# supranational/sppark

Hardware: NVIDIA H100
Metric: BLS12-381 G1 MSM/s @2^26 points (higher is better)
Workload: dtype u32x12 (384-bit Montgomery integers)

## Files before the change

### sppark_b200/csrc/msm/msm.cuh

```cuda
#pragma once
#include "../util/gpu.cuh"
#include "msm_core.cuh"
#include "msm_pair.cuh"
#include "msm_table.cuh"

namespace msm {

#ifndef SPPARK_B200_ACC_THREADS
# define SPPARK_B200_ACC_THREADS 128
#endif
#ifndef SPPARK_B200_ACC_MIN_BLOCKS
# define SPPARK_B200_ACC_MIN_BLOCKS 3
#endif
constexpr uint32_t ACC_THREADS = SPPARK_B200_ACC_THREADS;
constexpr uint32_t HEAVY_THREADS = 128;

constexpr uint32_t HIST_THREADS = 1024;
constexpr uint32_t HIST_SMEM_WORDS = 56 * 1024;
constexpr uint32_t SORT_THREADS = 512;
constexpr uint32_t SORT_CAP = 24576;

template<class Load, class Visit>
__device__ uint32_t block_exclusive_scan(uint32_t len, Load load, Visit visit)
{
    __shared__ uint32_t warp_tot[32];
    const uint32_t lane = threadIdx.x & 31, wid = threadIdx.x >> 5, nw = blockDim.x >> 5;
    uint32_t carry = 0;
    for (uint32_t t0 = 0; t0 < len; t0 += 4 * blockDim.x) {
        const uint32_t b = t0 + 4 * threadIdx.x;
        uint32_t c[4];
#pragma unroll
        for (uint32_t k = 0; k < 4; k++) c[k] = b + k < len ? load(b + k) : 0;
        const uint32_t s = c[0] + c[1] + c[2] + c[3];
        uint32_t x = s;
#pragma unroll
        for (uint32_t d = 1; d < 32; d <<= 1) {
            const uint32_t y = __shfl_up_sync(0xffffffffu, x, d);
            if (lane >= d) x += y;
        }
        if (lane == 31) warp_tot[wid] = x;
        __syncthreads();
        if (wid == 0) {
            uint32_t t = lane < nw ? warp_tot[lane] : 0;
#pragma unroll
            for (uint32_t d = 1; d < 32; d <<= 1) {
                const uint32_t y = __shfl_up_sync(0xffffffffu, t, d);
                if (lane >= d) t += y;
            }
            warp_tot[lane] = t;
        }
        __syncthreads();
        uint32_t r = carry + (wid ? warp_tot[wid - 1] : 0) + x - s;
        carry += warp_tot[31];
#pragma unroll
        for (uint32_t k = 0; k < 4; k++) {
            if (b + k < len) visit(b + k, c[k], r);
            r += c[k];
        }
        __syncthreads();
    }
    return carry;
}

static __global__ void __launch_bounds__(HIST_THREADS)
bin_hist_kernel(const Config cfg, uint32_t lg_bins, const uint32_t* scalars, uint32_t wpg, uint32_t* bin_count)
{
    extern __shared__ uint32_t hist[];
    const uint32_t w0 = blockIdx.y * wpg, w1 = min(w0 + wpg, cfg.nwins), nctr = (w1 - w0) << lg_bins;
    const uint32_t d_end = cfg.copies > 1 ? digit_count(cfg) : w1;
    const uint32_t lane = threadIdx.x & 31;
    for (uint32_t k = threadIdx.x; k < nctr; k += blockDim.x) hist[k] = 0;
    __syncthreads();
    for (uint32_t i0 = blockIdx.x * blockDim.x + (threadIdx.x & ~31u); i0 < cfg.npoints; i0 += gridDim.x * blockDim.x) {
        const uint32_t i = i0 + lane;
        for_each_digit(cfg, lg_bins, scalars, i, i < cfg.npoints, d_end,
                       [&](uint32_t w, bool nz, uint32_t bin, uint32_t, uint32_t) {
            if (w < w0 || w >= w1) return;
            const uint32_t key = nz ? bin - (w0 << lg_bins) : ~0u;
            const uint32_t peers = __match_any_sync(0xffffffffu, key);
            if (nz && lane == __ffs(peers) - 1) atomicAdd(&hist[key], __popc(peers));
        });
    }
    __syncthreads();
    for (uint32_t k = threadIdx.x; k < nctr; k += blockDim.x)
        if (hist[k]) atomicAdd(&bin_count[((size_t)w0 << lg_bins) + k], hist[k]);
}

static __global__ void __launch_bounds__(1024)
bin_scan_kernel(uint32_t lg_bins, const uint32_t* bin_count, uint32_t* bin_base, uint32_t* bin_cur)
{
    const size_t row = (size_t)blockIdx.x << lg_bins;
    block_exclusive_scan(1u << lg_bins, [&](uint32_t j) { return bin_count[row + j]; },
                         [&](uint32_t j, uint32_t, uint32_t off) { bin_base[row + j] = off; bin_cur[row + j] = off; });
}

static __global__ void __launch_bounds__(256)
partition_kernel(const Config cfg, uint32_t lg_bins, const uint32_t* scalars, uint32_t* bin_cur, uint2* staging)
{
    const uint32_t lane = threadIdx.x & 31;
    for (uint32_t i0 = blockIdx.x * blockDim.x + (threadIdx.x & ~31u); i0 < cfg.npoints; i0 += gridDim.x * blockDim.x) {
        const uint32_t i = i0 + lane;
        for_each_digit(cfg, lg_bins, scalars, i, i < cfg.npoints, digit_count(cfg),
                       [&](uint32_t w, bool nz, uint32_t bin, uint32_t b, uint32_t entry) {
            const uint32_t peers = __match_any_sync(0xffffffffu, nz ? bin : ~0u);
            const uint32_t leader = __ffs(peers) - 1;
            uint32_t pos = 0;
            if (nz && lane == leader) pos = atomicAdd(&bin_cur[bin], __popc(peers));
            pos = __shfl_sync(0xffffffffu, pos, leader) + __popc(peers & ((1u << lane) - 1));
            if (nz) staging[(size_t)w * row_stride(cfg) + pos] = make_uint2(entry, b);
        });
    }
}

static __global__ void __launch_bounds__(SORT_THREADS)
bin_sort_kernel(const Config cfg, uint32_t lg_bins, uint32_t cap, const uint2* staging, const uint32_t* bin_count,
                const uint32_t* bin_base, uint32_t* counts, uint32_t* offsets, uint32_t* sorted, uint32_t* ctrl,
                uint32_t* heavy_list, uint32_t* chunk_map, uint32_t* overflow)
{
    extern __shared__ uint32_t sm[];
    const uint32_t w = blockIdx.x >> lg_bins, bin = blockIdx.x & ((1u << lg_bins) - 1);
    uint32_t b0, nbk;
    if (!bin_buckets(cfg, lg_bins, w, bin, b0, nbk)) return;
    const uint32_t cnt = bin_count[blockIdx.x], base = bin_base[blockIdx.x];
    const size_t t0 = ((size_t)w << cfg.lg_nb) + b0;
    if (last_bin(cfg, lg_bins, w, bin))
        for (uint32_t b = b0 + nbk + threadIdx.x; b < (1u << cfg.lg_nb); b += blockDim.x)
            offsets[((size_t)w << cfg.lg_nb) + b] = base + cnt;
    if (cnt > cap) {
        if (threadIdx.x == 0) overflow[atomicAdd(&ctrl[3], 1)] = blockIdx.x;
        return;
    }
    uint32_t *run = sm, *cur = sm + cap;
    for (uint32_t k = threadIdx.x; k < nbk; k += blockDim.x) cur[k] = 0;
    __syncthreads();
    const uint2* src = staging + (size_t)w * row_stride(cfg) + base;
    for (uint32_t k = threadIdx.x; k < cnt; k += blockDim.x) atomicAdd(&cur[src[k].y - b0], 1);
    __syncthreads();
    block_exclusive_scan(nbk, [&](uint32_t j) { return cur[j]; }, [&](uint32_t j, uint32_t c, uint32_t off) {
        counts[t0 + j] = c;
        offsets[t0 + j] = base + off;
        cur[j] = off;
        register_heavy(cfg, (uint32_t)(t0 + j), c, ctrl, heavy_list, chunk_map);
    });
    for (uint32_t k = threadIdx.x; k < cnt; k += blockDim.x) {
        const uint2 e = src[k];
        run[atomicAdd(&cur[e.y - b0], 1)] = e.x;
    }
    __syncthreads();
    uint32_t* dst = sorted + (size_t)w * row_stride(cfg) + base;
    for (uint32_t k = threadIdx.x; k < cnt; k += blockDim.x) dst[k] = run[k];
}

template<bool PLACE>
__global__ void __launch_bounds__(256)
overflow_kernel(const Config cfg, uint32_t lg_bins, const uint2* staging, const uint32_t* bin_count,
                const uint32_t* bin_base, const uint32_t* ctrl, const uint32_t* overflow, uint32_t* slots,
                uint32_t* sorted)
{
    const uint32_t lane = threadIdx.x & 31, nov = ctrl[3];
    for (uint32_t o = 0; o < nov; o++) {
        const uint32_t g = overflow[o], w = g >> lg_bins, cnt = bin_count[g];
        const uint2* src = staging + (size_t)w * row_stride(cfg) + bin_base[g];
        uint32_t* row = slots + ((size_t)w << cfg.lg_nb);
        for (uint32_t k0 = blockIdx.x * blockDim.x + (threadIdx.x & ~31u); k0 < cnt; k0 += gridDim.x * blockDim.x) {
            const uint32_t k = k0 + lane;
            const uint2 e = k < cnt ? src[k] : make_uint2(0, ~0u);
            const uint32_t peers = __match_any_sync(0xffffffffu, e.y);
            const uint32_t leader = __ffs(peers) - 1;
            uint32_t pos = 0;
            if (k < cnt && lane == leader) pos = atomicAdd(&row[e.y], __popc(peers));
            if (PLACE) {
                pos = __shfl_sync(0xffffffffu, pos, leader) + __popc(peers & ((1u << lane) - 1));
                if (k < cnt) sorted[(size_t)w * row_stride(cfg) + pos] = e.x;
            }
        }
    }
}

static __global__ void __launch_bounds__(1024)
overflow_scan_kernel(const Config cfg, uint32_t lg_bins, const uint32_t* bin_base, const uint32_t* overflow,
                     const uint32_t* counts, uint32_t* offsets, uint32_t* cursor, uint32_t* ctrl,
                     uint32_t* heavy_list, uint32_t* chunk_map)
{
    const uint32_t nov = ctrl[3];
    for (uint32_t o = blockIdx.x; o < nov; o += gridDim.x) {
        const uint32_t g = overflow[o], w = g >> lg_bins, base = bin_base[g];
        uint32_t b0, nbk;
        bin_buckets(cfg, lg_bins, w, g & ((1u << lg_bins) - 1), b0, nbk);
        const size_t t0 = ((size_t)w << cfg.lg_nb) + b0;
        block_exclusive_scan(nbk, [&](uint32_t j) { return counts[t0 + j]; }, [&](uint32_t j, uint32_t c, uint32_t off) {
            offsets[t0 + j] = base + off;
            cursor[t0 + j] = base + off;
            register_heavy(cfg, (uint32_t)(t0 + j), c, ctrl, heavy_list, chunk_map);
        });
    }
}

struct SortBufs {
    uint32_t *counts, *offsets, *cursor, *ctrl, *heavy_list, *chunk_map, *sorted;
    uint32_t *bin_count, *bin_base, *bin_cur, *overflow;
    uint2* staging;
};

inline bool sort_profile() { const char* e = getenv("SPPARK_B200_MSM_SORT_PROFILE"); return e && atoi(e) != 0; }

inline void sort_slice(const Config& cfg, uint32_t cap, const uint32_t* d_scalars, const SortBufs& s, uint32_t sms,
                       cudaStream_t stream)
{
    const uint32_t lg_bins = sort_lg_bins(cfg, row_stride(cfg));
    const size_t nbins = (size_t)cfg.nwins << lg_bins, nslots = (size_t)cfg.nwins << cfg.lg_nb;
    const bool marks = sort_profile();
    CUDA_OK(cudaFuncSetAttribute(bin_hist_kernel, cudaFuncAttributeMaxDynamicSharedMemorySize, HIST_SMEM_WORDS * 4));
    CUDA_OK(cudaFuncSetAttribute(bin_sort_kernel, cudaFuncAttributeMaxDynamicSharedMemorySize,
                                 (SORT_CAP + (1u << SORT_SMAX)) * 4));
    CUDA_OK(cudaMemsetAsync(s.counts, 0, nslots * 4, stream));
    CUDA_OK(cudaMemsetAsync(s.ctrl, 0, 16, stream));
    CUDA_OK(cudaMemsetAsync(s.bin_count, 0, nbins * 4, stream));
    const uint32_t wpg = std::min(cfg.nwins, HIST_SMEM_WORDS >> lg_bins);
    const uint32_t ngroups = (cfg.nwins + wpg - 1) / wpg;
    const uint32_t hist_blk = (uint32_t)std::min<size_t>((cfg.npoints + HIST_THREADS - 1) / HIST_THREADS, sms);
    bin_hist_kernel<<<dim3(hist_blk, ngroups), HIST_THREADS, ((size_t)wpg << lg_bins) * 4, stream>>>(
        cfg, lg_bins, d_scalars, wpg, s.bin_count);
    COUNT_LAUNCH();
    bin_scan_kernel<<<cfg.nwins, 1024, 0, stream>>>(lg_bins, s.bin_count, s.bin_base, s.bin_cur);
    COUNT_LAUNCH();
    if (marks) g_profile.mark("sort_partition", stream);
    const uint32_t part_blk = (uint32_t)std::min<size_t>((cfg.npoints + 255) / 256, (size_t)sms * 8);
    partition_kernel<<<part_blk, 256, 0, stream>>>(cfg, lg_bins, d_scalars, s.bin_cur, s.staging);
    COUNT_LAUNCH();
    if (marks) g_profile.mark("sort_bins", stream);
    bin_sort_kernel<<<(uint32_t)nbins, SORT_THREADS, (cap + (1u << SORT_SMAX)) * 4, stream>>>(
        cfg, lg_bins, cap, s.staging, s.bin_count, s.bin_base, s.counts, s.offsets, s.sorted, s.ctrl,
        s.heavy_list, s.chunk_map, s.overflow);
    COUNT_LAUNCH();
    if (marks) g_profile.mark("sort_overflow", stream);
    overflow_kernel<false><<<sms * 4, 256, 0, stream>>>(cfg, lg_bins, s.staging, s.bin_count, s.bin_base, s.ctrl,
                                                        s.overflow, s.counts, s.sorted);
    overflow_scan_kernel<<<sms, 1024, 0, stream>>>(cfg, lg_bins, s.bin_base, s.overflow, s.counts, s.offsets, s.cursor,
                                                   s.ctrl, s.heavy_list, s.chunk_map);
    overflow_kernel<true><<<sms * 4, 256, 0, stream>>>(cfg, lg_bins, s.staging, s.bin_count, s.bin_base, s.ctrl,
                                                       s.overflow, s.cursor, s.sorted);
    COUNT_LAUNCH(); COUNT_LAUNCH(); COUNT_LAUNCH();
    CUDA_OK(cudaGetLastError());
}

static __global__ void pair_counts_kernel(const Config cfg, const uint32_t* counts, uint32_t* counts1, uint32_t nslots)
{
    for (uint32_t t = blockIdx.x * blockDim.x + threadIdx.x; t < nslots; t += gridDim.x * blockDim.x)
        pair_counts_body(cfg, counts, counts1, t);
}

static __global__ void __launch_bounds__(1024)
pair_scan_kernel(const Config cfg, const uint32_t* counts1, uint32_t* off1, uint32_t* wintotal)
{
    __shared__ uint32_t warp_tot[32];
    const uint32_t w = blockIdx.x, nb = 1u << cfg.lg_nb, lane = threadIdx.x & 31, wid = threadIdx.x >> 5;
    const size_t base = (size_t)w << cfg.lg_nb;
    uint32_t carry = 0;
    for (uint32_t t0 = 0; t0 < nb; t0 += 4096) {
        const uint32_t b = t0 + threadIdx.x * 4;
        uint4 c = make_uint4(0, 0, 0, 0);
        if (b < nb) c = *reinterpret_cast<const uint4*>(counts1 + base + b);
        const uint32_t s = c.x + c.y + c.z + c.w;
        uint32_t x = s;
#pragma unroll
        for (uint32_t d = 1; d < 32; d <<= 1) {
            uint32_t y = __shfl_up_sync(0xffffffffu, x, d);
            if (lane >= d) x += y;
        }
        if (lane == 31) warp_tot[wid] = x;
        __syncthreads();
        if (wid == 0) {
            uint32_t t = warp_tot[lane];
#pragma unroll
            for (uint32_t d = 1; d < 32; d <<= 1) {
                uint32_t y = __shfl_up_sync(0xffffffffu, t, d);
                if (lane >= d) t += y;
            }
            warp_tot[lane] = t;
        }
        __syncthreads();
        uint4 r;
        r.x = carry + (wid ? warp_tot[wid - 1] : 0) + x - s;
        r.y = r.x + c.x;
        r.z = r.y + c.y;
        r.w = r.z + c.z;
        carry += warp_tot[31];
        if (b < nb) *reinterpret_cast<uint4*>(off1 + base + b) = r;
        __syncthreads();
    }
    if (threadIdx.x == 0) wintotal[w] = carry;
}

static __global__ void pair_winbase_kernel(const Config cfg, const uint32_t* wintotal, uint32_t* winbase)
{
    if (blockIdx.x || threadIdx.x) return;
    uint32_t run = 0;
    for (uint32_t w = 0; w < cfg.nwins; w++) { winbase[w] = run; run += wintotal[w]; }
    winbase[cfg.nwins] = run;
}

template<class F>
__global__ void __launch_bounds__(128)
pair_forward_kernel(const Config cfg, const uint32_t* points, const uint32_t* sorted, const uint32_t* offsets,
                    const uint32_t* counts, const uint32_t* counts1, const uint32_t* off1, const uint32_t* winbase,
                    uint32_t o0, uint32_t nthreads, uint32_t* pre, uint32_t* totals)
{
    const uint32_t tid = blockIdx.x * blockDim.x + threadIdx.x;
    if (tid < nthreads)
        pair_forward_body<F>(cfg, points, sorted, offsets, counts, counts1, off1, winbase, o0, nthreads, pre, totals, tid);
}

// ... 249 lines not shown
finish_par_kernel(const Config cfg, const uint32_t* winR, uint32_t* out_jacobian)
{
    __shared__ F slots[Par4<F>::NS];
    if (threadIdx.x >= 4) return;
    Par4<F> p(slots, slots + 4, threadIdx.x);
    {
        const ec::xyzz_t<F> top = load_bucket<F>(winR, cfg.nwins - 1);
        if (p.lane == 0) { slots[Par4<F>::sX] = top.X; slots[Par4<F>::sY] = top.Y; slots[Par4<F>::sZZZ] = top.ZZZ; slots[Par4<F>::sZZ] = top.ZZ; }
        p.sync();
    }
    for (uint32_t w = cfg.nwins - 1; w-- > 0;) {
        for (uint32_t d = 0; d < cfg.wbits; d++) p.dbl();
        p.add(load_bucket<F>(winR, w));
    }
    const bool inf = p.is_inf();
    const F ZZ = slots[Par4<F>::sZZ];
    const F Yf = slots[Par4<F>::sY], ZZZf = slots[Par4<F>::sZZZ];
    const F r = F::mul_shared(p.pick(slots[Par4<F>::sX], Yf, Yf, Yf), p.pick(ZZ, ZZZf, ZZZf, ZZZf));
    if (p.lane < 2)
        for (int k = 0; k < F::N; k++) out_jacobian[p.lane * F::N + k] = inf ? 0 : r.l[k];
    if (p.lane == 2)
        for (int k = 0; k < F::N; k++) out_jacobian[2 * F::N + k] = inf ? 0 : ZZ.l[k];
}

static __global__ void pack_points_kernel(const uint8_t* in, size_t stride, uint32_t words, bool has_flag,
                                   uint32_t* out, uint32_t npoints)
{
    for (uint32_t i = blockIdx.x * blockDim.x + threadIdx.x; i < npoints; i += gridDim.x * blockDim.x) {
        const uint32_t* src = reinterpret_cast<const uint32_t*>(in + (size_t)i * stride);
        bool inf = has_flag && (in[(size_t)i * stride + 4 * words] & 1);
        for (uint32_t k = 0; k < words; k++) out[(size_t)i * words + k] = inf ? 0 : src[k];
    }
}

template<class F>
__global__ void __launch_bounds__(128)
table_double_kernel(const uint32_t* packed, size_t first, uint32_t n, uint32_t steps, uint32_t copies,
                    uint32_t* xyzz, uint32_t* zzz)
{
    const uint32_t i = blockIdx.x * blockDim.x + threadIdx.x;
    if (i < n) table_double_body<F>(packed, first, n, steps, copies, xyzz, zzz, i);
}

template<class F>
__global__ void __launch_bounds__(128)
table_normalize_kernel(const uint32_t* xyzz, const uint32_t* zzz_inv, size_t npoints, size_t first, uint32_t n,
                       uint32_t nslots, uint32_t* table)
{
    const uint32_t s = blockIdx.x * blockDim.x + threadIdx.x;
    if (s < nslots) table_normalize_body<F>(xyzz, zzz_inv, npoints, first, n, table, s);
}

template<class F>
void build_table(uint32_t* d_table, size_t npoints, const Config& cfg, const stream_t& stream)
{
    const uint32_t K1 = cfg.copies - 1, steps = cfg.wbits * cfg.nwins;
    if (K1 == 0 || npoints == 0) return;
    const size_t chunk = std::min<size_t>(npoints, ((size_t)1 << 21) / K1);
    dev_ptr_t<uint32_t> xyzz(chunk * K1 * 4 * F::N, stream), zzz(chunk * K1 * F::N, stream);
    for (size_t first = 0; first < npoints; first += chunk) {
        const uint32_t n = (uint32_t)std::min(chunk, npoints - first), ns = n * K1;
        table_double_kernel<F><<<(n + 127) / 128, 128, 0, stream>>>(d_table, first, n, steps, cfg.copies, xyzz, zzz);
        pair_invert_kernel<F><<<((ns + PAIR_M - 1) / PAIR_M + 127) / 128, 128, 0, stream>>>(zzz, ns);
        table_normalize_kernel<F><<<(ns + 127) / 128, 128, 0, stream>>>(xyzz, zzz, npoints, first, n, ns, d_table);
        COUNT_LAUNCH(); COUNT_LAUNCH(); COUNT_LAUNCH();
        CUDA_OK(cudaGetLastError());
    }
}

template<class F>
class msm_t {
    const gpu_t& gpu;
    static constexpr uint32_t PW = 2 * F::N, BW = 4 * F::N, JW = 3 * F::N;

public:
    explicit msm_t(const gpu_t& g) : gpu(g) {}

    struct Job {
        Config cfg;
        size_t nslots, slice_cap;
        uint32_t lg_l, items1;
        uint8_t* blob;
        uint32_t *counts, *offsets, *cursor, *ctrl, *heavy_list, *chunk_map, *partials, *sorted, *buckets;
        uint32_t *bin_count, *bin_base, *bin_cur, *overflow;
        uint2* staging;
        uint32_t *R[2], *S[2];
        uint32_t slices_done;
        bool pair;
        size_t pair_bound;
        uint32_t pair_threads;
        uint32_t *counts1, *off1, *wintotal, *winbase, *sums, *pre, *totals;
        cudaStream_t owner;
        Job() : blob(nullptr), owner(nullptr) {}
        Job(const Job&) = delete;
        Job& operator=(const Job&) = delete;
        Job(Job&& o) noexcept { memcpy((void*)this, (const void*)&o, sizeof(Job)); o.blob = nullptr; }
        ~Job() { if (blob) (void)cudaFreeAsync(blob, owner); }
    };

    Job begin(size_t total_points, size_t slice_cap, cudaStream_t stream)
    {
        if (total_points >= (1ull << 31))
            throw cuda_error(-(int)cudaErrorInvalidValue, "msm: npoints must be < 2^31");
        return begin(make_config(total_points), slice_cap, stream);
    }

    Job begin(const Config& cfg, size_t slice_cap, cudaStream_t stream)
    {
        Job j;
        j.cfg = cfg;
        j.cfg.npoints = (uint32_t)slice_cap;
        j.slice_cap = slice_cap;
        j.nslots = (size_t)j.cfg.nwins << j.cfg.lg_nb;
        j.lg_l = j.cfg.lg_nb > 12 ? j.cfg.lg_nb - 12 : 0;
        j.items1 = j.cfg.nwins << (j.cfg.lg_nb - j.lg_l);
        j.slices_done = 0;
        const size_t entries = (size_t)j.cfg.nwins * row_stride(j.cfg);
        const size_t heavy_cap = entries / (j.cfg.heavy + 1) + 1;
        const size_t chunk_cap = entries / j.cfg.heavy_chunk + heavy_cap;
        size_t off = 0;
        auto take = [&](size_t bytes) { size_t o = off; off += (bytes + 255) & ~(size_t)255; return o; };
        const size_t o_counts = take(j.nslots * 4), o_offsets = take(j.nslots * 4), o_cursor = take(j.nslots * 4);
        const size_t nbins = (size_t)j.cfg.nwins << sort_lg_bins(j.cfg, row_stride(j.cfg));
        const size_t o_bcount = take(nbins * 4), o_bbase = take(nbins * 4), o_bcur = take(nbins * 4), o_over = take(nbins * 4);
        const size_t o_staging = take(entries * 8);
        const size_t o_ctrl = take(16), o_heavy = take(heavy_cap * 12), o_cmap = take(chunk_cap * 4);
        const size_t o_partials = take(chunk_cap * BW * 4);
        const size_t o_sorted = take(entries * 4);
        const size_t o_buckets = take(j.nslots * BW * 4);
        const size_t o_r0 = take((size_t)j.items1 * BW * 4), o_s0 = take((size_t)j.items1 * BW * 4);
        const size_t o_r1 = take((size_t)j.items1 * BW * 4 / 2 + 4096), o_s1 = take((size_t)j.items1 * BW * 4 / 2 + 4096);
        const char* pair_env = getenv("SPPARK_B200_MSM_PAIR");
        j.pair = pair_env && atoi(pair_env) != 0 && entries + j.nslots < (1ull << 31);
        j.pair_bound = (entries + std::min<size_t>(entries, j.nslots) + 1) / 2;
        j.pair_threads = (uint32_t)std::min<size_t>((j.pair_bound + PAIR_K - 1) / PAIR_K, (size_t)1 << 21);
        size_t o_c1 = 0, o_o1 = 0, o_wt = 0, o_wb = 0, o_sums = 0, o_pre = 0, o_tot = 0;
        if (j.pair) {
            o_c1 = take(j.nslots * 4); o_o1 = take(j.nslots * 4);
            o_wt = take((j.cfg.nwins + 1) * 4); o_wb = take((j.cfg.nwins + 1) * 4);
            o_sums = take(j.pair_bound * 2 * F::N * 4);
            o_pre = take((size_t)j.pair_threads * PAIR_K * F::N * 4);
            o_tot = take((size_t)j.pair_threads * F::N * 4);
        }
        CUDA_OK(cudaMallocAsync((void**)&j.blob, off, stream));
        j.owner = stream;
        auto U32 = [&](size_t o) { return reinterpret_cast<uint32_t*>(j.blob + o); };
        j.counts = U32(o_counts); j.offsets = U32(o_offsets); j.cursor = U32(o_cursor);
        j.ctrl = U32(o_ctrl); j.heavy_list = U32(o_heavy); j.chunk_map = U32(o_cmap);
        j.partials = U32(o_partials); j.sorted = U32(o_sorted); j.buckets = U32(o_buckets);
        j.bin_count = U32(o_bcount); j.bin_base = U32(o_bbase); j.bin_cur = U32(o_bcur); j.overflow = U32(o_over);
        j.staging = reinterpret_cast<uint2*>(j.blob + o_staging);
        j.R[0] = U32(o_r0); j.S[0] = U32(o_s0); j.R[1] = U32(o_r1); j.S[1] = U32(o_s1);
        j.counts1 = U32(o_c1); j.off1 = U32(o_o1); j.wintotal = U32(o_wt); j.winbase = U32(o_wb);
        j.sums = U32(o_sums); j.pre = U32(o_pre); j.totals = U32(o_tot);
        g_profile.reset();
        return j;
    }

    void slice(Job& j, const uint32_t* d_points, const uint32_t* d_scalars, size_t n, cudaStream_t stream)
    {
        if (n == 0) return;
        Config cfg = j.cfg;
        cfg.npoints = (uint32_t)n;
        cfg.merge = j.slices_done ? 1 : 0;
        const uint32_t sms = (uint32_t)gpu.sm_count();
        g_profile.mark("sort", stream);
        const SortBufs sb{j.counts, j.offsets, j.cursor, j.ctrl, j.heavy_list, j.chunk_map, j.sorted,
                          j.bin_count, j.bin_base, j.bin_cur, j.overflow, j.staging};
        sort_slice(cfg, SORT_CAP, d_scalars, sb, sms, stream);

        g_profile.mark("accumulate", stream);
        int occ = 1;
        CUDA_OK(cudaOccupancyMaxActiveBlocksPerMultiprocessor(&occ, accumulate_kernel<F>, ACC_THREADS, 0));
        if (occ < 1) occ = 1;
        size_t want = (j.nslots + ACC_THREADS - 1) / ACC_THREADS;
        uint32_t acc_blocks = (uint32_t)std::min<size_t>(want, (size_t)sms * occ);
        if (j.pair) {
            const uint32_t nslots = (uint32_t)j.nslots;
            pair_counts_kernel<<<sms * 8, 256, 0, stream>>>(cfg, j.counts, j.counts1, nslots);
            pair_scan_kernel<<<cfg.nwins, 1024, 0, stream>>>(cfg, j.counts1, j.off1, j.wintotal);
            pair_winbase_kernel<<<1, 32, 0, stream>>>(cfg, j.wintotal, j.winbase);
            const size_t ent = (size_t)cfg.nwins * row_stride(cfg);
            const size_t bound = (ent + std::min<size_t>(ent, j.nslots) + 1) / 2;
            const size_t per_launch = (size_t)j.pair_threads * PAIR_K;
            for (size_t o0 = 0; o0 < bound; o0 += per_launch) {
                const uint32_t nth = (uint32_t)std::min<size_t>(j.pair_threads, (bound - o0 + PAIR_K - 1) / PAIR_K);
                pair_forward_kernel<F><<<(nth + 127) / 128, 128, 0, stream>>>(
                    cfg, d_points, j.sorted, j.offsets, j.counts, j.counts1, j.off1, j.winbase, (uint32_t)o0, nth, j.pre, j.totals);
                pair_invert_kernel<F><<<((nth + PAIR_M - 1) / PAIR_M + 127) / 128, 128, 0, stream>>>(j.totals, nth);
                pair_backward_kernel<F><<<(nth + 127) / 128, 128, 0, stream>>>(
                    cfg, d_points, j.sorted, j.offsets, j.counts, j.counts1, j.off1, j.winbase, (uint32_t)o0, nth, j.pre, j.totals, j.sums);
                COUNT_LAUNCH(); COUNT_LAUNCH(); COUNT_LAUNCH();
            }
            CUDA_OK(cudaGetLastError());
            g_profile.mark("accumulate_sums", stream);
            accumulate_direct_kernel<F><<<acc_blocks, ACC_THREADS, 0, stream>>>(cfg, j.sums, j.offsets, j.counts, j.buckets,
                                                                               j.ctrl, j.counts1, j.off1, j.winbase);
        } else {
            accumulate_kernel<F><<<acc_blocks, ACC_THREADS, 0, stream>>>(cfg, d_points, j.sorted, j.offsets, j.counts,
                                                                        j.buckets, j.ctrl);
        }
        COUNT_LAUNCH();
        g_profile.mark("heavy", stream);
        heavy_chunks_kernel<F><<<sms * 4, HEAVY_THREADS, HEAVY_THREADS * BW * 4, stream>>>(
            cfg, d_points, j.sorted, j.offsets, j.counts, j.ctrl, j.heavy_list, j.chunk_map, j.partials);
        COUNT_LAUNCH();
        heavy_fold_kernel<F><<<sms, HEAVY_THREADS, HEAVY_THREADS * BW * 4, stream>>>(cfg, j.ctrl, j.heavy_list,
                                                                                    j.partials, j.buckets);
        COUNT_LAUNCH();
        CUDA_OK(cudaGetLastError());
        if (getenv("SPPARK_B200_MSM_DEBUG")) {
            uint32_t dbg[3];
            CUDA_OK(cudaMemcpyAsync(dbg, j.ctrl, 12, cudaMemcpyDeviceToHost, stream));
            CUDA_OK(cudaStreamSynchronize(stream));
            fprintf(stderr, "[msm] slice %u n=%u wbits=%u nwins=%u heavy_thr=%u tasks_claimed=%u nheavy=%u nchunks=%u acc_blocks=%u"
                    " digits=%u sets=%u copies=%u\n",
                    j.slices_done, cfg.npoints, cfg.wbits, cfg.nwins, cfg.heavy, dbg[0], dbg[1], dbg[2], acc_blocks,
                    digit_count(cfg), cfg.nwins, cfg.copies);
        }
        j.slices_done++;
    }

    void finish(Job& j, uint32_t* d_out, cudaStream_t stream)
    {
        if (j.slices_done == 0) {
            CUDA_OK(cudaMemsetAsync(d_out, 0, JW * 4, stream));
        } else {
            const Config& cfg = j.cfg;
            g_profile.mark("reduce", stream);
            reduce1_kernel<F><<<(j.items1 + 127) / 128, 128, 0, stream>>>(cfg, j.buckets, j.lg_l, j.items1, j.R[0], j.S[0]);
            COUNT_LAUNCH();
            uint32_t per_win = 1u << (cfg.lg_nb - j.lg_l), lg_span = j.lg_l, cur = 0;
            while (per_win > 1) {
                uint32_t lg_g = 31 - __builtin_clz(per_win);
                if (lg_g > 4) lg_g = 4;
                uint32_t G = 1u << lg_g, nitems = cfg.nwins * (per_win >> lg_g);
                constexpr uint32_t PG = par_groups<F>::value;
                combine_par_kernel<F><<<(nitems + PG - 1) / PG, 4 * PG, 0, stream>>>(j.R[cur], j.S[cur], G, lg_span, nitems,
                                                                                     j.R[cur ^ 1], j.S[cur ^ 1]);
                COUNT_LAUNCH();
                per_win >>= lg_g;
                lg_span += lg_g;
                cur ^= 1;
            }
            g_profile.mark("finish", stream);
            finish_par_kernel<F><<<1, 32, 0, stream>>>(cfg, j.R[cur], d_out);
            COUNT_LAUNCH();
            g_profile.mark("end", stream);
            CUDA_OK(cudaGetLastError());
        }
        CUDA_OK(cudaFreeAsync(j.blob, stream));
// ... 18 lines not shown
```

### sppark_b200/csrc/msm/msm_bls12_381.cu

```cuda
#include "msm_host.cuh"

RustError msm_host_bls12_381(void* out, const void* points, size_t npoints, const void* scalars,
                             size_t stride, bool has_flag, bool mont)
{
    return msm_host<ff::bls12_381_fp_t>(out, points, npoints, scalars, stride, has_flag,
                                        mont ? scalars_from_mont<ff::bls12_381_fr_t> : nullptr);
}
RustError msm_dev_bls12_381(void* out, const void* d_points, size_t npoints, const void* d_scalars, void* stream)
{   return msm_dev<ff::bls12_381_fp_t>(out, d_points, npoints, d_scalars, stream);   }

RustError gen_points_bls12_381(void* d_out, size_t n, void* stream)
{   return gen_points_dev<ff::bls12_381_g1_gen>(d_out, n, stream);   }
RustError combine_bls12_381(void* out, const void* partials, size_t count)
{   return combine_host<ff::bls12_381_fp_t>(out, partials, count);   }

extern "C" RustError mult_pippenger(void* out, const void* points, size_t npoints, const void* scalars)
{   return msm_host_bls12_381(out, points, npoints, scalars, 96, false, false);   }

extern "C" RustError mult_pippenger_inf(void* out, const void* points, size_t npoints,
                                        const void* scalars, size_t ffi_affine_sz)
{   return msm_host_bls12_381(out, points, npoints, scalars, ffi_affine_sz, true, false);   }

template<class F>
__global__ void selftest_kernel(int op, size_t n, uint32_t* r, const uint32_t* a, const uint32_t* b)
{
    size_t i = blockIdx.x * (size_t)blockDim.x + threadIdx.x;
    if (i >= n) return;
    F x, y, z;
    for (int k = 0; k < F::N; k++) { x.l[k] = a[i * F::N + k]; y.l[k] = b[i * F::N + k]; }
    switch (op) {
    case 0: z = x * y; break;
    case 1: z = x + y; break;
    case 2: z = x - y; break;
    case 3: z = x.sqr(); break;
    case 4: z = F::mul_shared(x, y); break;
    case 5: z = F::sqr_shared(x); break;
    default: z = F::msub_shared(x, y, y, x.sqr()); break;
    }
    for (int k = 0; k < F::N; k++) r[i * F::N + k] = z.l[k];
}

template<class F>
static RustError selftest(int op, size_t n, void* r, const void* a, const void* b)
{
    try {
        const gpu_t& gpu = select_gpu(-1);
        const stream_t& s = gpu[0];
        size_t bytes = n * F::N * 4;
        dev_ptr_t<uint32_t> da(n * F::N, s), db(n * F::N, s), dr(n * F::N, s);
        s.HtoD(da, a, bytes);
        s.HtoD(db, b, bytes);
        selftest_kernel<F><<<(unsigned)((n + 127) / 128), 128, 0, s>>>(op, n, dr, da, db);
        COUNT_LAUNCH();
        CUDA_OK(cudaGetLastError());
        s.DtoH(r, dr, bytes);
        s.sync();
    } catch (const cuda_error& e) {
        return rust_err(e.code(), e.what());
    }
    return rust_ok();
}

extern "C" RustError sppark_b200_selftest_field(int field, int op, size_t n, void* r, const void* a, const void* b)
{
    switch (field) {
    case 0: return selftest<ff::bls12_381_fp_t>(op, n, r, a, b);
    case 1: return selftest<ff::bls12_381_fr_t>(op, n, r, a, b);
    case 2: return selftest<ff::pallas_fp_t>(op, n, r, a, b);
    case 3: return selftest<ff::vesta_fp_t>(op, n, r, a, b);
    case 4: return selftest<ff::bn254_fp_t>(op, n, r, a, b);
    case 5: return selftest<ff::bn254_fr_t>(op, n, r, a, b);
    case 6: return selftest<ff::bls12_377_fp_t>(op, n, r, a, b);
    case 7: return selftest<ff::bls12_377_fr_t>(op, n, r, a, b);
    default: return rust_err(-(int)cudaErrorInvalidValue, "selftest: unknown field");
    }
}

RustError msm_preload_bls12_381(const void* points, size_t npoints, size_t stride, bool has_flag, void** d_points,
                                uint32_t* copies, uint32_t* wbits)
{   return msm_preload<ff::bls12_381_fp_t>(points, npoints, stride, has_flag, d_points, copies, wbits);   }
RustError msm_resident_bls12_381(void* out, const void* d_points, size_t npoints, const void* scalars, bool mont,
                                 uint32_t wbits, uint32_t copies, size_t stride)
{
    return msm_resident<ff::bls12_381_fp_t, ff::bls12_381_fr_t>(out, d_points, npoints, scalars, mont, wbits, copies, stride);
}

extern "C" RustError sppark_b200_selftest_msm_sort(size_t n, uint32_t wbits, uint32_t cap, const void* scalars,
                                                   void* counts, void* offsets, void* sorted, void* heavy_slots,
                                                   uint32_t* info)
{
    using namespace msm;
    if (n == 0 || n >= (1ull << 31) || wbits < 3 || wbits > 24 || cap > SORT_CAP)
        return rust_err(-(int)cudaErrorInvalidValue, "selftest_msm_sort: bad arguments");
    try {
        const gpu_t& gpu = select_gpu(-1);
        const stream_t& s = gpu[0];
        Config cfg = make_config(n);
        cfg.wbits = wbits;
        cfg.nwins = (256 + wbits - 1) / wbits;
        cfg.lg_nb = wbits - 1;
        const size_t nslots = (size_t)cfg.nwins << cfg.lg_nb, entries = (size_t)cfg.nwins * n;
        const size_t nbins = (size_t)cfg.nwins << sort_lg_bins(cfg, n);
        const size_t heavy_cap = entries / (cfg.heavy + 1) + 1, chunk_cap = entries / cfg.heavy_chunk + heavy_cap;
        dev_ptr_t<uint32_t> d_sc(8 * n, s), d_counts(nslots, s), d_offsets(nslots, s), d_cursor(nslots, s);
        dev_ptr_t<uint32_t> d_ctrl(4, s), d_heavy(3 * heavy_cap, s), d_cmap(chunk_cap, s), d_sorted(entries, s);
        dev_ptr_t<uint32_t> d_bcount(nbins, s), d_bbase(nbins, s), d_bcur(nbins, s), d_over(nbins, s);
        dev_ptr_t<uint32_t> d_staging(2 * entries, s);
        s.HtoD(d_sc, scalars, 32 * n);
        const SortBufs sb{d_counts, d_offsets, d_cursor, d_ctrl, d_heavy, d_cmap, d_sorted,
                          d_bcount, d_bbase, d_bcur, d_over, reinterpret_cast<uint2*>((uint32_t*)d_staging)};
        sort_slice(cfg, cap ? cap : SORT_CAP, d_sc, sb, (uint32_t)gpu.sm_count(), s);
        uint32_t ctrl[4];
        s.DtoH(ctrl, d_ctrl, 16);
        s.DtoH(counts, d_counts, nslots * 4);
        s.DtoH(offsets, d_offsets, nslots * 4);
        s.DtoH(sorted, d_sorted, entries * 4);
        s.sync();
        std::vector<uint32_t> hl(3 * (size_t)ctrl[1] + 1);
        if (ctrl[1]) s.DtoH(hl.data(), d_heavy, 12 * (size_t)ctrl[1]);
        s.sync();
        for (uint32_t h = 0; h < ctrl[1]; h++) static_cast<uint32_t*>(heavy_slots)[h] = hl[3 * h];
        info[0] = cfg.nwins; info[1] = cfg.heavy; info[2] = ctrl[1]; info[3] = sort_lg_bins(cfg, n); info[4] = ctrl[3];
    } catch (const cuda_error& e) {
        return rust_err(e.code(), e.what());
    }
    return rust_ok();
}
```

### sppark_b200/csrc/msm/msm_core.cuh

```cuda
#pragma once
#include <algorithm>
#include "../ec/xyzz.cuh"

namespace msm {

struct Config {
    uint32_t wbits;
    uint32_t nwins;
    uint32_t lg_nb;
    uint32_t npoints;
    uint32_t heavy;
    uint32_t heavy_chunk;
    uint32_t merge;
    uint32_t copies;
    uint32_t copy_stride;
};

HD uint32_t digit_count(const Config& cfg) { return (256 + cfg.wbits - 1) / cfg.wbits; }
HD size_t row_stride(const Config& cfg) { return cfg.copies * cfg.npoints; }

HD uint32_t digit_slot(const Config& cfg, uint32_t w, uint32_t i, uint32_t neg, uint32_t& entry)
{
    if (cfg.copies == 1) { entry = i | (neg << 31); return w; }
    const uint32_t k = w / cfg.nwins;
// ... 38 lines not shown
            carry = 1;
            raw = (1u << c) - raw;
        } else {
            neg = 0;
            carry = 0;
        }
        bucket = raw - 1;
        return raw != 0;
    }
};

HD void count_body(const Config& cfg, const uint32_t* scalars, uint32_t* counts, uint32_t i)
{
    Digits d(scalars + 8 * (size_t)i);
    const uint32_t nd = digit_count(cfg);
    for (uint32_t w = 0; w < nd; w++) {
        uint32_t b, neg, entry;
        if (d.next(w, cfg.wbits, b, neg))
            atomic_inc(&counts[((size_t)digit_slot(cfg, w, i, neg, entry) << cfg.lg_nb) + b]);
    }
}

HD void scatter_body(const Config& cfg, const uint32_t* scalars, uint32_t* cursor,
                     uint32_t* sorted, uint32_t i, uint32_t w0, uint32_t w1)
{
    Digits d(scalars + 8 * (size_t)i);
    for (uint32_t w = 0; w < w1; w++) {
        uint32_t b, neg, entry;
        if (d.next(w, cfg.wbits, b, neg) && w >= w0) {
            const uint32_t v = digit_slot(cfg, w, i, neg, entry);
            uint32_t pos = atomic_inc(&cursor[((size_t)v << cfg.lg_nb) + b]);
            sorted[(size_t)v * row_stride(cfg) + pos] = entry;
        }
    }
}

constexpr uint32_t SORT_SMAX = 12;
constexpr uint32_t SORT_LG_FILL = 13;

HD uint32_t top_window_bits(const Config& cfg)
{
    const uint32_t e = 255 - (cfg.nwins - 1) * cfg.wbits;
    return e < cfg.lg_nb ? e : cfg.lg_nb;
}
HD uint32_t window_bits(const Config& cfg, uint32_t w)
{   return w + 1 < cfg.nwins || cfg.copies > 1 ? cfg.lg_nb : top_window_bits(cfg);   }
HD uint32_t bin_shift(const Config& cfg, uint32_t lg_bins, uint32_t w)
{
    const uint32_t ub = window_bits(cfg, w);
    return ub > lg_bins ? ub - lg_bins : 0;
}

inline uint32_t sort_lg_bins(const Config& cfg, size_t n)
{
    int lg_n = 0;
    while (((size_t)1 << lg_n) < n) lg_n++;
    int lb = std::max(std::min(lg_n - (int)SORT_LG_FILL, 15), (int)cfg.lg_nb - (int)SORT_SMAX);
    lb = std::min(lb, (int)cfg.lg_nb);
    return (uint32_t)std::max(lb, 2);
}

HD bool bin_buckets(const Config& cfg, uint32_t lg_bins, uint32_t w, uint32_t bin, uint32_t& b0, uint32_t& nbk)
{
    const uint32_t s = bin_shift(cfg, lg_bins, w), ub = window_bits(cfg, w);
    b0 = bin << s;
    nbk = 1u << s;
    return b0 < (1u << ub);
}

HD bool last_bin(const Config& cfg, uint32_t lg_bins, uint32_t w, uint32_t bin)
{   return ((bin + 1) << bin_shift(cfg, lg_bins, w)) == (1u << window_bits(cfg, w));   }

template<class Fn>
HD void for_each_digit(const Config& cfg, uint32_t lg_bins, const uint32_t* scalars, uint32_t i, bool valid,
                       uint32_t w_end, Fn fn)
{
    Digits d(scalars + 8 * (size_t)(valid ? i : 0));
    for (uint32_t w = 0; w < w_end; w++) {
        uint32_t b, neg, entry;
        const bool nz = d.next(w, cfg.wbits, b, neg) && valid;
        const uint32_t v = digit_slot(cfg, w, i, neg, entry);
        fn(v, nz, (v << lg_bins) + (nz ? b >> bin_shift(cfg, lg_bins, v) : 0), b, entry);
    }
}

HD void register_heavy(const Config& cfg, uint32_t t, uint32_t cnt, uint32_t* ctrl, uint32_t* heavy_list,
                       uint32_t* chunk_map)
{
    if (cnt <= cfg.heavy) return;
    const uint32_t h = atomic_inc(&ctrl[1]), nch = (cnt + cfg.heavy_chunk - 1) / cfg.heavy_chunk;
    const uint32_t first_chunk = atomic_inc(&ctrl[2], nch);
    heavy_list[3 * h] = t;
    heavy_list[3 * h + 1] = first_chunk;
    heavy_list[3 * h + 2] = nch;
    for (uint32_t q = 0; q < nch; q++) chunk_map[first_chunk + q] = h;
}

template<class F>
HD ec::affine_t<F> load_point(const uint32_t* points, uint32_t entry)
{
    constexpr int W = 2 * F::N;
    const uint32_t* p = points + (size_t)(entry & 0x7fffffffu) * W;
    ec::affine_t<F> a;
#if defined(__CUDA_ARCH__)
    static_assert(W % 4 == 0, "affine point must be a whole number of 16-byte words");
    uint32_t buf[W];
#pragma unroll
    for (int k = 0; k < W / 4; k++) {
        uint4 v = __ldg(reinterpret_cast<const uint4*>(p) + k);
        buf[4 * k] = v.x; buf[4 * k + 1] = v.y; buf[4 * k + 2] = v.z; buf[4 * k + 3] = v.w;
    }
#pragma unroll
    for (int k = 0; k < F::N; k++) { a.X.l[k] = buf[k]; a.Y.l[k] = buf[F::N + k]; }
#else
    for (int k = 0; k < F::N; k++) { a.X.l[k] = p[k]; a.Y.l[k] = p[F::N + k]; }
#endif
    if (entry >> 31) a.Y = a.Y.neg();
    return a;
}

template<class F>
HD void store_bucket(uint32_t* buckets, size_t slot, const ec::xyzz_t<F>& b)
{
    constexpr int W = 4 * F::N;
    uint32_t* p = buckets + slot * W;
#pragma unroll
    for (int k = 0; k < F::N; k++) {
        p[k] = b.X.l[k]; p[F::N + k] = b.Y.l[k]; p[2 * F::N + k] = b.ZZZ.l[k]; p[3 * F::N + k] = b.ZZ.l[k];
    }
}

template<class F>
HD ec::xyzz_t<F> load_bucket(const uint32_t* buckets, size_t slot)
{
    constexpr int W = 4 * F::N;
    const uint32_t* p = buckets + slot * W;
    ec::xyzz_t<F> b;
#pragma unroll
    for (int k = 0; k < F::N; k++) {
        b.X.l[k] = p[k]; b.Y.l[k] = p[F::N + k]; b.ZZZ.l[k] = p[2 * F::N + k]; b.ZZ.l[k] = p[3 * F::N + k];
    }
    return b;
}

template<class F, bool DIRECT = false>
HD void accumulate_body(const Config& cfg, const uint32_t* points, const uint32_t* sorted,
                        const uint32_t* offsets, const uint32_t* counts, uint32_t* buckets,
                        uint32_t* task_counter, const uint32_t* counts1 = nullptr,
                        const uint32_t* off1 = nullptr, const uint32_t* winbase = nullptr)
{
    const uint32_t total = cfg.nwins << cfg.lg_nb;
    ec::xyzz_t<F> acc;
    const uint32_t* run = nullptr;
    uint32_t t = 0, k = 0, cnt = 0, direct_base = 0;
    bool open = false, live = true;
    for (;;) {
        if (live && k == cnt) {
            if (open) store_bucket<F>(buckets, t, acc);
            open = false;
            for (;;) {
                t = atomic_inc(task_counter);
                if (t >= total) { live = false; break; }
                t = total - 1 - t;
                cnt = counts[t];
                if (cnt == 0) {
                    if (!cfg.merge) {
// ... 154 lines not shown
```

Baseline: 2.403.

## Replace scattered partition with two-pass shared-memory coarse/fine partition

Replaces the single-pass partition kernel, which scattered each digit entry to global memory through per-bin atomics, with a two-level radix partition. A coarse pass bins tiles of points in shared memory by coarse key and writes contiguous runs. A fine pass then splits each coarse chunk into the final bins, again staging in shared memory before coalesced writes. The goal is fewer uncoalesced scattered stores and less global atomic traffic, at the cost of an extra read/write pass over the entries and an extra coarse buffer that aliases the sorted buffer.

```diff
diff --git a/sppark_b200/csrc/msm/msm.cuh b/sppark_b200/csrc/msm/msm.cuh
--- a/sppark_b200/csrc/msm/msm.cuh
+++ b/sppark_b200/csrc/msm/msm.cuh
@@ -87,29 +87,147 @@
 }
 
 static __global__ void __launch_bounds__(1024)
-bin_scan_kernel(uint32_t lg_bins, const uint32_t* bin_count, uint32_t* bin_base, uint32_t* bin_cur)
+bin_scan_kernel(uint32_t lg_bins, uint32_t q, uint32_t chunk, const uint32_t* bin_count, uint32_t* bin_base,
+                uint32_t* bin_cur, uint32_t* coarse_cur, uint32_t* coarse_chunk)
 {
     const size_t row = (size_t)blockIdx.x << lg_bins;
     block_exclusive_scan(1u << lg_bins, [&](uint32_t j) { return bin_count[row + j]; },
                          [&](uint32_t j, uint32_t, uint32_t off) { bin_base[row + j] = off; bin_cur[row + j] = off; });
-}
-
-static __global__ void __launch_bounds__(256)
-partition_kernel(const Config cfg, uint32_t lg_bins, const uint32_t* scalars, uint32_t* bin_cur, uint2* staging)
+    if (q == 0) return;
+    const uint32_t nco = 1u << (lg_bins - q), v = blockIdx.x;
+    uint32_t* cf = coarse_chunk + (size_t)v * (nco + 1);
+    const uint32_t total = block_exclusive_scan(nco, [&](uint32_t cb) {
+        uint32_t lo, hi;
+        coarse_range(lg_bins, q, bin_base, bin_count, v, cb, lo, hi);
+        return (hi - lo + chunk - 1) / chunk;
+    }, [&](uint32_t cb, uint32_t, uint32_t off) {
+        cf[cb] = off;
+        coarse_cur[((size_t)v << (lg_bins - q)) + cb] = bin_base[row + (cb << q)];
+    });
+    if (threadIdx.x == 0) cf[nco] = total;
+}
+
+constexpr uint32_t PART_THREADS = 512;
+constexpr uint32_t PART_ENTS = 12288, PART_TILE_MIN = 896, PART_LG_RUN = 4;
+constexpr size_t PART_SMEM = PART_ENTS * 8 + 3 * PART_KEYS * 4;
+
+DEV uint32_t warp_claim(uint32_t* ctr, uint32_t key, bool on)
 {
     const uint32_t lane = threadIdx.x & 31;
-    for (uint32_t i0 = blockIdx.x * blockDim.x + (threadIdx.x & ~31u); i0 < cfg.npoints; i0 += gridDim.x * blockDim.x) {
-        const uint32_t i = i0 + lane;
-        for_each_digit(cfg, lg_bins, scalars, i, i < cfg.npoints, digit_count(cfg),
-                       [&](uint32_t w, bool nz, uint32_t bin, uint32_t b, uint32_t entry) {
-            const uint32_t peers = __match_any_sync(0xffffffffu, nz ? bin : ~0u);
-            const uint32_t leader = __ffs(peers) - 1;
-            uint32_t pos = 0;
-            if (nz && lane == leader) pos = atomicAdd(&bin_cur[bin], __popc(peers));
-            pos = __shfl_sync(0xffffffffu, pos, leader) + __popc(peers & ((1u << lane) - 1));
-            if (nz) staging[(size_t)w * row_stride(cfg) + pos] = make_uint2(entry, b);
+    uint32_t left = __ballot_sync(0xffffffffu, on), pos = 0;
+#pragma unroll
+    for (int r = 0; r < 2; r++) {
+        if (!left) break;
+        const uint32_t leader = __ffs(left) - 1, k = __shfl_sync(0xffffffffu, key, leader);
+        const uint32_t peers = __ballot_sync(0xffffffffu, ((left >> lane) & 1) && key == k);
+        uint32_t base = 0;
+        if (lane == leader) base = atomicAdd(&ctr[k], __popc(peers));
+        base = __shfl_sync(0xffffffffu, base, leader);
+        if ((peers >> lane) & 1) pos = base + __popc(peers & ((1u << lane) - 1));
+        left &= ~peers;
+    }
+    if ((left >> lane) & 1) pos = atomicAdd(&ctr[key], 1);
+    return pos;
+}
+
+DEV void part_write_out(const Config& cfg, uint32_t w0, uint32_t lgk, uint32_t nkeys, uint32_t total,
+                        const uint2* ent, const uint32_t* loc, const uint32_t* gbase, uint2* dst)
+{
+    for (uint32_t p = threadIdx.x; p < total; p += blockDim.x) {
+        const uint32_t k = run_of(loc, nkeys, p);
+        dst[(size_t)(w0 + (k >> lgk)) * row_stride(cfg) + gbase[k] + (p - loc[k])] = ent[p];
+    }
+}
+
+static __global__ void __launch_bounds__(PART_THREADS, 2)
+partition_coarse_kernel(const Config cfg, uint32_t lg_bins, PartPlan pp, const uint32_t* scalars, uint32_t* cur,
+                        uint2* dst)
+{
+    extern __shared__ uint2 ent[];
+    uint32_t* hist = reinterpret_cast<uint32_t*>(ent + PART_ENTS);
+    uint32_t *loc = hist + PART_KEYS, *gbase = loc + PART_KEYS;
+    const uint32_t lane = threadIdx.x & 31, lgc = lg_bins - pp.q;
+    const uint32_t t0 = blockIdx.x * pp.tile, t1 = min(t0 + pp.tile, cfg.npoints);
+    for (uint32_t w0 = 0; w0 < cfg.nwins; w0 += pp.sets) {
+        const uint32_t w1 = min(w0 + pp.sets, cfg.nwins), nkeys = (w1 - w0) << lgc;
+        const uint32_t d_end = cfg.copies > 1 ? digit_count(cfg) : w1;
+        for (uint32_t k = threadIdx.x; k < nkeys; k += blockDim.x) hist[k] = 0;
+        __syncthreads();
+        for (uint32_t i0 = t0 + (threadIdx.x & ~31u); i0 < t1; i0 += blockDim.x) {
+            const uint32_t i = i0 + lane;
+            for_each_digit(cfg, lg_bins, scalars, i, i < t1, d_end, [&](uint32_t w, bool nz, uint32_t bin, uint32_t, uint32_t) {
+                if (w < w0 || w >= w1) return;
+                warp_claim(hist, (bin - (w0 << lg_bins)) >> pp.q, nz);
+            });
+        }
+        __syncthreads();
+        const uint32_t total = block_exclusive_scan(nkeys, [&](uint32_t k) { return hist[k]; },
+                                                    [&](uint32_t k, uint32_t c, uint32_t off) {
+            loc[k] = hist[k] = off;
+            if (c) gbase[k] = atomicAdd(&cur[((size_t)w0 << lgc) + k], c);
         });
-    }
+        for (uint32_t i0 = t0 + (threadIdx.x & ~31u); i0 < t1; i0 += blockDim.x) {
+            const uint32_t i = i0 + lane;
+            for_each_digit(cfg, lg_bins, scalars, i, i < t1, d_end, [&](uint32_t w, bool nz, uint32_t bin, uint32_t b, uint32_t entry) {
+                if (w < w0 || w >= w1) return;
+                const uint32_t pos = warp_claim(hist, (bin - (w0 << lg_bins)) >> pp.q, nz);
+                if (nz) ent[pos] = make_uint2(entry, b);
+            });
+        }
+        __syncthreads();
+        part_write_out(cfg, w0, lgc, nkeys, total, ent, loc, gbase, dst);
+        __syncthreads();
+    }
+}
+
+static __global__ void __launch_bounds__(PART_THREADS, 2)
+partition_fine_kernel(const Config cfg, uint32_t lg_bins, PartPlan pp, const uint32_t* bin_count,
+                      const uint32_t* bin_base, const uint32_t* coarse_chunk, uint32_t* bin_cur, const uint2* coarse,
+                      uint2* staging)
+{
+    extern __shared__ uint2 ent[];
+    uint32_t* hist = reinterpret_cast<uint32_t*>(ent + PART_ENTS);
+    uint32_t *loc = hist + PART_KEYS, *gbase = loc + PART_KEYS;
+    const uint32_t v = blockIdx.y, lane = threadIdx.x & 31, nkeys = 1u << pp.q, s = bin_shift(cfg, lg_bins, v);
+    uint32_t cb, k0, k1;
+    if (!part_chunk(lg_bins, pp.q, pp.chunk, bin_base, bin_count, coarse_chunk, v, blockIdx.x, cb, k0, k1)) return;
+    const uint2* src = coarse + (size_t)v * row_stride(cfg);
+    for (uint32_t k = threadIdx.x; k < nkeys; k += blockDim.x) hist[k] = 0;
+    __syncthreads();
+    constexpr uint32_t U = 4;
+    for (uint32_t j0 = k0 + (threadIdx.x & ~31u) * U; j0 < k1; j0 += blockDim.x * U) {
+        uint32_t key[U];
+#pragma unroll
+        for (uint32_t u = 0; u < U; u++) {
+            const uint32_t j = j0 + 32 * u + lane;
+            key[u] = j < k1 ? (src[j].y >> s) & (nkeys - 1) : 0;
+        }
+#pragma unroll
+        for (uint32_t u = 0; u < U; u++) warp_claim(hist, key[u], j0 + 32 * u + lane < k1);
+    }
+    __syncthreads();
+    const size_t fine0 = ((size_t)v << lg_bins) + (cb << pp.q);
+    const uint32_t total = block_exclusive_scan(nkeys, [&](uint32_t k) { return hist[k]; },
+                                                [&](uint32_t k, uint32_t c, uint32_t off) {
+        loc[k] = hist[k] = off;
+        if (c) gbase[k] = atomicAdd(&bin_cur[fine0 + k], c);
+    });
+    for (uint32_t j0 = k0 + (threadIdx.x & ~31u) * U; j0 < k1; j0 += blockDim.x * U) {
+        uint2 e[U];
+#pragma unroll
+        for (uint32_t u = 0; u < U; u++) {
+            const uint32_t j = j0 + 32 * u + lane;
+            e[u] = j < k1 ? src[j] : make_uint2(0, 0);
+        }
+#pragma unroll
+        for (uint32_t u = 0; u < U; u++) {
+            const bool on = j0 + 32 * u + lane < k1;
+            const uint32_t pos = warp_claim(hist, (e[u].y >> s) & (nkeys - 1), on);
+            if (on) ent[pos] = e[u];
+        }
+    }
+    __syncthreads();
+    part_write_out(cfg, v, pp.q, nkeys, total, ent, loc, gbase, staging);
 }
 
 static __global__ void __launch_bounds__(SORT_THREADS)
@@ -199,7 +317,9 @@
 struct SortBufs {
     uint32_t *counts, *offsets, *cursor, *ctrl, *heavy_list, *chunk_map, *sorted;
     uint32_t *bin_count, *bin_base, *bin_cur, *overflow;
+    uint32_t *coarse_cur, *coarse_chunk;
     uint2* staging;
+    uint2* coarse;
 };
 
 inline bool sort_profile() { const char* e = getenv("SPPARK_B200_MSM_SORT_PROFILE"); return e && atoi(e) != 0; }
@@ -222,12 +342,23 @@
     bin_hist_kernel<<<dim3(hist_blk, ngroups), HIST_THREADS, ((size_t)wpg << lg_bins) * 4, stream>>>(
         cfg, lg_bins, d_scalars, wpg, s.bin_count);
     COUNT_LAUNCH();
-    bin_scan_kernel<<<cfg.nwins, 1024, 0, stream>>>(lg_bins, s.bin_count, s.bin_base, s.bin_cur);
+    const PartPlan pp = part_plan(cfg, lg_bins, PART_ENTS, PART_TILE_MIN, PART_LG_RUN);
+    bin_scan_kernel<<<cfg.nwins, 1024, 0, stream>>>(lg_bins, pp.q, pp.chunk, s.bin_count, s.bin_base, s.bin_cur,
+                                                    s.coarse_cur, s.coarse_chunk);
     COUNT_LAUNCH();
-    if (marks) g_profile.mark("sort_partition", stream);
-    const uint32_t part_blk = (uint32_t)std::min<size_t>((cfg.npoints + 255) / 256, (size_t)sms * 8);
-    partition_kernel<<<part_blk, 256, 0, stream>>>(cfg, lg_bins, d_scalars, s.bin_cur, s.staging);
+    CUDA_OK(cudaFuncSetAttribute(partition_coarse_kernel, cudaFuncAttributeMaxDynamicSharedMemorySize, PART_SMEM));
+    CUDA_OK(cudaFuncSetAttribute(partition_fine_kernel, cudaFuncAttributeMaxDynamicSharedMemorySize, PART_SMEM));
+    if (marks) g_profile.mark("sort_partition_coarse", stream);
+    partition_coarse_kernel<<<(cfg.npoints + pp.tile - 1) / pp.tile, PART_THREADS, PART_SMEM, stream>>>(
+        cfg, lg_bins, pp, d_scalars, pp.q ? s.coarse_cur : s.bin_cur, pp.q ? s.coarse : s.staging);
     COUNT_LAUNCH();
+    if (marks) g_profile.mark("sort_partition_fine", stream);
+    if (pp.q) {
+        const size_t chunks = (row_stride(cfg) + pp.chunk - 1) / pp.chunk + ((size_t)1 << (lg_bins - pp.q));
+        partition_fine_kernel<<<dim3((uint32_t)chunks, cfg.nwins), PART_THREADS, PART_SMEM, stream>>>(
+            cfg, lg_bins, pp, s.bin_count, s.bin_base, s.coarse_chunk, s.bin_cur, s.coarse, s.staging);
+        COUNT_LAUNCH();
+    }
     if (marks) g_profile.mark("sort_bins", stream);
     bin_sort_kernel<<<(uint32_t)nbins, SORT_THREADS, (cap + (1u << SORT_SMAX)) * 4, stream>>>(
         cfg, lg_bins, cap, s.staging, s.bin_count, s.bin_base, s.counts, s.offsets, s.sorted, s.ctrl,
@@ -643,8 +774,9 @@
         uint32_t lg_l, items1;
         uint8_t* blob;
         uint32_t *counts, *offsets, *cursor, *ctrl, *heavy_list, *chunk_map, *partials, *sorted, *buckets;
-        uint32_t *bin_count, *bin_base, *bin_cur, *overflow;
+        uint32_t *bin_count, *bin_base, *bin_cur, *overflow, *coarse_cur, *coarse_chunk;
         uint2* staging;
+        uint2* coarse;
         uint32_t *R[2], *S[2];
         uint32_t slices_done;
         bool pair;
@@ -684,10 +816,11 @@
         const size_t o_counts = take(j.nslots * 4), o_offsets = take(j.nslots * 4), o_cursor = take(j.nslots * 4);
         const size_t nbins = (size_t)j.cfg.nwins << sort_lg_bins(j.cfg, row_stride(j.cfg));
         const size_t o_bcount = take(nbins * 4), o_bbase = take(nbins * 4), o_bcur = take(nbins * 4), o_over = take(nbins * 4);
+        const size_t o_ccur = take(nbins * 4), o_cchunk = take((nbins + j.cfg.nwins) * 4);
         const size_t o_staging = take(entries * 8);
         const size_t o_ctrl = take(16), o_heavy = take(heavy_cap * 12), o_cmap = take(chunk_cap * 4);
         const size_t o_partials = take(chunk_cap * BW * 4);
-        const size_t o_sorted = take(entries * 4);
+        const size_t o_coarse = take(entries * 8), o_sorted = o_coarse;
         const size_t o_buckets = take(j.nslots * BW * 4);
         const size_t o_r0 = take((size_t)j.items1 * BW * 4), o_s0 = take((size_t)j.items1 * BW * 4);
         const size_t o_r1 = take((size_t)j.items1 * BW * 4 / 2 + 4096), o_s1 = take((size_t)j.items1 * BW * 4 / 2 + 4096);
@@ -710,7 +843,9 @@
         j.ctrl = U32(o_ctrl); j.heavy_list = U32(o_heavy); j.chunk_map = U32(o_cmap);
         j.partials = U32(o_partials); j.sorted = U32(o_sorted); j.buckets = U32(o_buckets);
         j.bin_count = U32(o_bcount); j.bin_base = U32(o_bbase); j.bin_cur = U32(o_bcur); j.overflow = U32(o_over);
+        j.coarse_cur = U32(o_ccur); j.coarse_chunk = U32(o_cchunk);
         j.staging = reinterpret_cast<uint2*>(j.blob + o_staging);
+        j.coarse = reinterpret_cast<uint2*>(j.blob + o_coarse);
         j.R[0] = U32(o_r0); j.S[0] = U32(o_s0); j.R[1] = U32(o_r1); j.S[1] = U32(o_s1);
         j.counts1 = U32(o_c1); j.off1 = U32(o_o1); j.wintotal = U32(o_wt); j.winbase = U32(o_wb);
         j.sums = U32(o_sums); j.pre = U32(o_pre); j.totals = U32(o_tot);
@@ -727,7 +862,8 @@
         const uint32_t sms = (uint32_t)gpu.sm_count();
         g_profile.mark("sort", stream);
         const SortBufs sb{j.counts, j.offsets, j.cursor, j.ctrl, j.heavy_list, j.chunk_map, j.sorted,
-                          j.bin_count, j.bin_base, j.bin_cur, j.overflow, j.staging};
+                          j.bin_count, j.bin_base, j.bin_cur, j.overflow, j.coarse_cur, j.coarse_chunk,
+                          j.staging, j.coarse};
         sort_slice(cfg, SORT_CAP, d_scalars, sb, sms, stream);
 
         g_profile.mark("accumulate", stream);
diff --git a/sppark_b200/csrc/msm/msm_bls12_381.cu b/sppark_b200/csrc/msm/msm_bls12_381.cu
--- a/sppark_b200/csrc/msm/msm_bls12_381.cu
+++ b/sppark_b200/csrc/msm/msm_bls12_381.cu
@@ -105,10 +105,11 @@
         dev_ptr_t<uint32_t> d_sc(8 * n, s), d_counts(nslots, s), d_offsets(nslots, s), d_cursor(nslots, s);
         dev_ptr_t<uint32_t> d_ctrl(4, s), d_heavy(3 * heavy_cap, s), d_cmap(chunk_cap, s), d_sorted(entries, s);
         dev_ptr_t<uint32_t> d_bcount(nbins, s), d_bbase(nbins, s), d_bcur(nbins, s), d_over(nbins, s);
-        dev_ptr_t<uint32_t> d_staging(2 * entries, s);
+        dev_ptr_t<uint32_t> d_ccur(nbins, s), d_cchunk(nbins + cfg.nwins, s), d_staging(2 * entries, s), d_coarse(2 * entries, s);
         s.HtoD(d_sc, scalars, 32 * n);
         const SortBufs sb{d_counts, d_offsets, d_cursor, d_ctrl, d_heavy, d_cmap, d_sorted,
-                          d_bcount, d_bbase, d_bcur, d_over, reinterpret_cast<uint2*>((uint32_t*)d_staging)};
+                          d_bcount, d_bbase, d_bcur, d_over, d_ccur, d_cchunk,
+                          reinterpret_cast<uint2*>((uint32_t*)d_staging), reinterpret_cast<uint2*>((uint32_t*)d_coarse)};
         sort_slice(cfg, cap ? cap : SORT_CAP, d_sc, sb, (uint32_t)gpu.sm_count(), s);
         uint32_t ctrl[4];
         s.DtoH(ctrl, d_ctrl, 16);
diff --git a/sppark_b200/csrc/msm/msm_core.cuh b/sppark_b200/csrc/msm/msm_core.cuh
--- a/sppark_b200/csrc/msm/msm_core.cuh
+++ b/sppark_b200/csrc/msm/msm_core.cuh
@@ -144,6 +144,65 @@
         const uint32_t v = digit_slot(cfg, w, i, neg, entry);
         fn(v, nz, (v << lg_bins) + (nz ? b >> bin_shift(cfg, lg_bins, v) : 0), b, entry);
     }
+}
+
+constexpr uint32_t PART_KEYS = 1024;
+
+struct PartPlan {
+    uint32_t q;
+    uint32_t sets;
+    uint32_t tile;
+    uint32_t chunk;
+};
+
+inline PartPlan part_plan(const Config& cfg, uint32_t lg_bins, uint32_t ents, uint32_t tile_min, uint32_t lg_run)
+{
+    PartPlan p;
+    const uint32_t K = cfg.copies, V = cfg.nwins;
+    const uint32_t per = std::max(1u, std::min(V, ents / (K * tile_min)));
+    const uint32_t groups = (V + per - 1) / per;
+    p.sets = (V + groups - 1) / groups;
+    uint32_t lgc = 0;
+    while (lgc < lg_bins && ((ents / (p.sets * K)) >> (lgc + 1)) >= (1u << lg_run)) lgc++;
+    while ((lg_bins - lgc) > 10) lgc++;
+    if ((p.sets << lgc) > PART_KEYS) p.sets = PART_KEYS >> lgc;
+    p.q = lg_bins - lgc;
+    p.tile = (ents / (p.sets * K)) & ~31u;
+    p.chunk = ents;
+    return p;
+}
+
+HD uint32_t run_of(const uint32_t* first, uint32_t nkeys, uint32_t x)
+{
+    uint32_t lo = 0, hi = nkeys;
+    while (hi - lo > 1) {
+        const uint32_t mid = (lo + hi) >> 1;
+        if (first[mid] <= x) lo = mid;
+        else hi = mid;
+    }
+    return lo;
+}
+
+HD void coarse_range(uint32_t lg_bins, uint32_t q, const uint32_t* bin_base, const uint32_t* bin_count, uint32_t v,
+                     uint32_t cb, uint32_t& lo, uint32_t& hi)
+{
+    const size_t row = (size_t)v << lg_bins, last = row + ((cb + 1) << q) - 1;
+    lo = bin_base[row + (cb << q)];
+    hi = bin_base[last] + bin_count[last];
+}
+
+HD bool part_chunk(uint32_t lg_bins, uint32_t q, uint32_t chunk, const uint32_t* bin_base, const uint32_t* bin_count,
+                   const uint32_t* coarse_chunk, uint32_t v, uint32_t x, uint32_t& cb, uint32_t& k0, uint32_t& k1)
+{
+    const uint32_t nco = 1u << (lg_bins - q);
+    const uint32_t* cf = coarse_chunk + (size_t)v * (nco + 1);
+    if (x >= cf[nco]) return false;
+    cb = run_of(cf, nco, x);
+    uint32_t lo, hi;
+    coarse_range(lg_bins, q, bin_base, bin_count, v, cb, lo, hi);
+    k0 = lo + (x - cf[cb]) * chunk;
+    k1 = hi - k0 < chunk ? hi : k0 + chunk;
+    return true;
 }
 
 HD void register_heavy(const Config& cfg, uint32_t t, uint32_t cnt, uint32_t* ctrl, uint32_t* heavy_list,
```

Result: faster. 2.474, median of 6 (+3.0%).
